# jneem/nnnoiseless

Hardware: AMD Instinct MI355X
Metric: 480-sample frames/sec (whole node) at N concurrent streams (higher is better)
Workload: dtype f32; 1 GPU; configs[2]: 65536 concurrent streams on one GPU, built-in weights.rnn, GRU as batched MFMA GEMM, synthetic 48 kHz sine+noise, 48 frame(s) per stream per step; parity=oracle pinned by the reference's golden pair (built-in model), model=built-in weights.rnn, boundary_format=f32 planar (process_frame's own), streams_per_gpu=65536, streams_total=65536, inputs_ready=True, schedule=stages, lanes=2, parallelism=streams sharded x1, one process per GPU, no data-path collective

## Files before the change

nnnoiseless_amd/csrc/nnn_kernels.hip:

```cpp
#pragma once
#include "nnn_layout.h"
#include <nnn_mfma.h>

namespace nnn {

#define NNN_TI(ptr, len, tile, lane) ((ptr) + ((size_t)(tile) * (len)) * TILE + (lane))
#define NNN_TIF(b, field, len, f, tile, lane) ((b).field + ((size_t)(b).S_pad * (size_t)(f) + (size_t)(tile) * TILE) * (size_t)(len) + (lane))

#define NNN_FRAME_SPLIT(PER)                              \
    const int frame = (int)blockIdx.x / (int)(PER);      \
    const int bx = (int)blockIdx.x - frame * (int)(PER); \
    b = frame_view(b, frame);

__device__ __forceinline__ void xcd_tile_block(int blk, int ntiles, int bpt, int &tile, int &sub)
{
    const int m8 = ntiles & ~7;
    if (blk < m8 * bpt) {
        const int xcd = blk & 7, j = blk >> 3;
        tile = xcd + 8 * (j / bpt);
        sub = j % bpt;
    } else {
        const int r = blk - m8 * bpt;
        tile = m8 + r / bpt;
        sub = r % bpt;
    }
}
__device__ __forceinline__ void xcd_tile_block_units(int blk, int ntiles, int bpt, int n, int &unit, int &tile, int &sub)
{
    const int m8 = ntiles & ~7;
    if (blk < m8 * bpt * n) {
        const int xcd = blk & 7, j = blk >> 3, tb = j / n;
        unit = j - tb * n;
        tile = xcd + 8 * (tb / bpt);
        sub = tb % bpt;
    } else {
        const int r = blk - m8 * bpt * n, per = (ntiles - m8) * bpt;
        unit = r / per;
        const int q = r - unit * per;
        tile = m8 + q / bpt;
        sub = q % bpt;
    }
}

#ifdef NNN_STAMPS
#define NNN_STAMP(b, i) do { if (blockIdx.x == 0 && blockIdx.y == 0 && threadIdx.x == 0) (b).stamps[i] = (long long)__builtin_readcyclecounter(); } while (0)
#define NNN_STAMPW(b, i, cond) do { if (blockIdx.x == 0 && (threadIdx.x & 63) == 0 && (cond)) (b).stamps[i] = (long long)__builtin_readcyclecounter(); } while (0)
#ifndef NNN_WFSTAMP_PHASE
#define NNN_WFSTAMP_PHASE 1
#endif
#else
#define NNN_STAMP(b, i) do { } while (0)
#define NNN_STAMPW(b, i, cond) do { } while (0)
#endif

#ifdef __HIPCC__
#define NNN_CONSTANT static __constant__
#else
#define NNN_CONSTANT __constant__
#endif
NNN_CONSTANT int kEband[NB] = {0, 1, 2, 3, 4, 5, 6, 7, 8, 10, 12, 14, 16, 20, 24, 28, 34, 40, 48, 60, 78, 100};
NNN_CONSTANT int kSecondCheck[16] = {0, 0, 3, 2, 3, 2, 5, 2, 3, 2, 3, 2, 5, 2, 3, 2};

template <int FMT> __device__ __forceinline__ float pcm_load(const char *p)
{
    if (FMT == PCM_I16) return (float)ld_global<short>(p);
    const float v = ld_global<float>(p);
    return FMT == PCM_F32_UNIT ? v * 32768.0f : v;
}
__device__ __forceinline__ short pcm_to_i16(float v) { return (short)roundf(fminf(fmaxf(v, -32768.0f), 32767.0f)); }
__device__ __forceinline__ float pcm_to_unit(float v)
{
    v = v / 32768.0f;
    if (v < -1.0f) v = -1.0f;
    if (v > 1.0f) v = 1.0f;
    return v;
}
__device__ __forceinline__ void pcm_store(char *p, int fmt, float v)
{
    if (fmt == PCM_I16) *(short *)p = pcm_to_i16(v);
    else *(float *)p = fmt == PCM_F32_UNIT ? pcm_to_unit(v) : v;
}
#ifndef NNN_HP_CH
#define NNN_HP_CH 32
#endif
constexpr int HP_CH = NNN_HP_CH;
// ... 571 lines not shown
    const float x0 = NNN_TI(b.xlp0, b.nslot, tile, lane)[(size_t)slot * TILE];
    float a1[1];
    if (wave == 0) lpc_chains<0, 1, LPC_CHW>(base, x0, a1);
    else if (wave == 1) lpc_chains<1, 1, LPC_CHW>(base, x0, a1);
    else if (wave == 2) lpc_chains<2, 1, LPC_CHW>(base, x0, a1);
    else if (wave == 3) lpc_chains<3, 1, LPC_CHW>(base, x0, a1);
    else lpc_chains<4, 1, LPC_CHW>(base, x0, a1);
    acs[wave][lane] = a1[0];
    __syncthreads();
    if (wave != 0) return;
    float ac[5];
#pragma unroll
    for (int k = 0; k < 5; k++) ac[k] = acs[k][lane];
    lpc_finish(b, tile, lane, slot, ac);
}

constexpr int PK_SPB = 16;
constexpr int PK_WAVES = 8;
constexpr int PK_T = 64 * PK_WAVES;
#ifndef NNN_PK_LC
#define NNN_PK_LC 13
#endif
constexpr int PK_LC = NNN_PK_LC;
constexpr int PK_NG = (NLAG1 + PK_LC - 1) / PK_LC;
static_assert((PK_LC & 1) && PK_NG <= 4 * 8, "odd group size: neighbouring groups start on different row parities");
constexpr int PK_XW = (PK_NG + 3) / 4;
constexpr int PK_JB = 8;
constexpr int PK_NP = PK_LC / 2;
constexpr int PK_NT = PK_JB / 2 + PK_NP;
static_assert((PK_NG - 1) * PK_LC + 239 + PK_JB + PK_LC < XLP / 2, "the window stays inside the even rows");
constexpr int PK_KMAX = 12;
constexpr int PK_NE = 1 + 2 * (PK_KMAX - 1);
constexpr int PK_NSLOT = PK_NE + 2;
constexpr int PK_NC = 36;

constexpr int PK_HALF = (XLP / 2) * PK_SPB;
constexpr int PK_ODD = PK_HALF + 16;
__device__ __forceinline__ int pk_at(int r, int s) { return ((r & 1) ? PK_ODD : 0) + (r >> 1) * PK_SPB + s; }


struct BestPitch {
    float best_num, second_num, best_den, second_den;
    int best, second;
    __device__ void init() { best_num = -1.0f; second_num = -1.0f; best_den = 0.0f; second_den = 0.0f; best = 0; second = 1; }
    __device__ __forceinline__ void update(int i, float corr, float y_sq_norm) {
        const float num = corr * corr;
        const bool in = corr > 0.0f && num * second_den > second_num * y_sq_norm;
        const bool top = in && num * best_den > best_num * y_sq_norm;
        const bool mid = in && !top;
        second_num = top ? best_num : (mid ? num : second_num);
        second_den = top ? best_den : (mid ? y_sq_norm : second_den);
        second = top ? best : (mid ? i : second);
        best_num = top ? num : best_num;
        best_den = top ? y_sq_norm : best_den;
        best = top ? i : best;
    }
    __device__ __forceinline__ void update_sq(int i, float num, float y_sq_norm) {
        const bool in = num * second_den > second_num * y_sq_norm;
        if (!wave_any(in)) return;
        const bool top = in && num * best_den > best_num * y_sq_norm;
        const bool mid = in && !top;
        second_num = top ? best_num : (mid ? num : second_num);
        second_den = top ? best_den : (mid ? y_sq_norm : second_den);
        second = top ? best : (mid ? i : second);
        best_num = top ? num : best_num;
        best_den = top ? y_sq_norm : best_den;
// ... 26 lines not shown
constexpr int PK_RMAX = 24;
constexpr int PK_CAP = 384;
constexpr int PK_PLW = XLP / 2 + 8;
constexpr float PK_EPS = 0.0083f;
struct PkCert {
    float denck[PK_SPB][PK_DCK];
    float bsum[PK_SPB][27];
    unsigned mask[PK_SPB][5];
    unsigned count, full, pad_[2];
    unsigned short list[PK_CAP];
    float slotv[PK_SPB][PK_RMAX], slotd[PK_SPB][PK_RMAX];
    int slotl[PK_SPB][PK_RMAX];
    alignas(16) unsigned short plane[(PK_SPB / 2) * PK_PLW + 16];
};
struct alignas(16) PkLds {
    float pb[PK_ODD + PK_HALF];
    float ckf[PK_NCKF][PK_SPB];
    float cky[PK_NCKY][PK_SPB];
    union {
        struct { float xc[NLAG1][PK_SPB], ysq[NLAG1][PK_SPB]; } c;
        PkCert a;
        struct {
            float part[PK_NC][4][PK_SPB];
            float yy[32][PK_SPB];
            float ye[10][PK_SPB];
            int cand[32][PK_SPB];
            int lo[2][PK_SPB];
            int tsel[PK_SPB];
            float xx[PK_SPB], lgain[PK_SPB];
            int t0[PK_SPB], pprev[PK_SPB];
            float kxy[16][PK_SPB], kyy[16][PK_SPB], kg[16][PK_SPB];
            int kpass[16][PK_SPB];
            int any_refine;
        } f;
    } u;
};
static_assert(sizeof(PkLds) <= 80 * 1024, "two blocks per CU");
static_assert(offsetof(PkLds, ckf) % 16 == 0 && offsetof(PkLds, u) % 16 == 0 && offsetof(PkCert, plane) % 16 == 0 && (PK_PLW * 2) % 16 == 0, "16-byte fragment reads");
static_assert(sizeof(float) * (PK_NCKF + PK_NCKY) * PK_SPB >= sizeof(unsigned short) * (PK_SPB / 2) * PK_PLW + 32, "the first eight planes fit over the check points");

constexpr int PK_CH = 32, PK_NCH = XLP / PK_CH;
static_assert(PK_NCH * PK_CH == XLP && PK_NCH * PK_SPB <= PK_T, "");

__device__ __forceinline__ void pk_window_load(const Buffers &b, const StepParams *sp, int tile, int q0, int tid, float (&v)[PK_CH],
                                               float (&fir)[5])
{
    const int col = tid & 15, ch = tid >> 4;
    if (ch >= PK_NCH) {
#pragma unroll
        for (int i = 0; i < PK_CH; i++) v[i] = 0.0f;
#pragma unroll
        for (int i = 0; i < 5; i++) fir[i] = 0.0f;
        return;
    }
    const int slot = sp->slot;
    {
        const float *lp = NNN_TI(b.lpc, b.nslot * 10, tile, q0 + col) + (size_t)(slot * 10) * TILE;
#pragma unroll
        for (int i = 0; i < 5; i++) fir[i] = lp[(size_t)(5 + i) * TILE];
    }
    const float *base = b.dec + ((size_t)tile * dec_len(b.nslot) + (size_t)dec_base(slot, b.nslot)) * TILE + q0;
    const unsigned off = (unsigned)(ch * PK_CH) * TILE + (unsigned)col;
#pragma unroll
    for (int i = 0; i < PK_CH; i++) v[i] = base[off + (unsigned)i * TILE];
    if (ch == 0) v[0] = NNN_TI(b.xlp0, b.nslot, tile, q0 + col)[(size_t)slot * TILE];
}

template <int NCAND>
// ... 230 lines not shown
}

__device__ __forceinline__ float pk_dot240(const float *xp, const float *yp)
{
    float c = 0.0f;
    v2f xa[4], ya[4], xb[4], yb[4];
#define NNN_LD(X, Y, J) do { _Pragma("unroll") for (int i_ = 0; i_ < 4; i_++) { \
        X[i_] = mk2(xp[((J) + 2 * i_) * PK_SPB], xp[((J) + 2 * i_ + 1) * PK_SPB]); Y[i_] = mk2(yp[((J) + 2 * i_) * PK_SPB], yp[((J) + 2 * i_ + 1) * PK_SPB]); } } while (0)
#define NNN_ACC(X, Y) do { _Pragma("unroll") for (int i_ = 0; i_ < 4; i_++) { const v2f pr_ = pk_mul(X[i_], Y[i_]); c = sadd(c, pr_.x); c = sadd(c, pr_.y); } } while (0)
    NNN_LD(xa, ya, 0);
#pragma nounroll
    for (int j = 0; j < 224; j += 16) {
        NNN_LD(xb, yb, j + 8);
        NNN_ACC(xa, ya);
        NNN_LD(xa, ya, j + 16);
        NNN_ACC(xb, yb);
    }
    NNN_LD(xb, yb, 232);
    NNN_ACC(xa, ya);
    NNN_ACC(xb, yb);
#undef NNN_LD
#undef NNN_ACC
    return c;
}

constexpr int PK_SEG_FS = 120;
#ifndef NNN_PK_SEG_F1
#define NNN_PK_SEG_F1 44
#endif
constexpr int PK_SEG_F1 = NNN_PK_SEG_F1;
static_assert(PK_SEG_F1 % 2 == 0 && PK_SEG_F1 <= PK_FINE_K, "");


template <bool HELD> __device__ __forceinline__ void xt_rider(const Buffers &b, const StepParams *sp, int rb, void *lds);

#ifndef NNN_PK_MINWAVES
#define NNN_PK_MINWAVES 4
#endif
template <bool LPC, bool HELD = false>
__global__ void __launch_bounds__(PK_T, NNN_PK_MINWAVES) k_pitch(Buffers b, const StepParams *sp0, int g, int chain, int seq0, unsigned tbase, int lpc_here_,
                                                                 int riders)
{
    __shared__ PkLds L;
    const int lpc_here = LPC ? lpc_here_ : 0;
    if (riders > 0 && (int)blockIdx.x >= riders) {
        xt_rider<HELD>(b, sp0, (int)blockIdx.x - riders, &L);
        return;
    }
    const int wave = __builtin_amdgcn_readfirstlane((int)(threadIdx.x >> 6)), lane0 = threadIdx.x & 63;
    int lane = lane0, s = lane & 15, q = lane >> 4;
    int item = (int)blockIdx.x;
    if (chain) {
        if (threadIdx.x == 0) L.u.f.any_refine = (int)(ticket_take(b.ticket) - tbase);
        __syncthreads();
        item = __builtin_amdgcn_readfirstlane(L.u.f.any_refine);
        __syncthreads();
    }
    const int per = b.S_pad / PK_SPB;
    const int f_begin = chain ? item / per : 0, f_end = chain ? f_begin + 1 : g;
    int tile, sub_;
    xcd_tile_block(item - f_begin * per, b.NT, TILE / PK_SPB, tile, sub_);
    const int q0 = sub_ * PK_SPB;
    if (tile * TILE + q0 >= b.S) return;
    static_assert(PK_SPB == 16, "the block's bits of the tile's word are read as one little-endian 16-bit value");
    if (HELD && b.live && ((const unsigned short *)b.live)[tile * (TILE / PK_SPB) + sub_] == 0) return;
    const int min_period = PITCH_MIN / 2, max_period = PITCH_MAX / 2;
    const bool dec_lane = wave == 0 && lane0 < PK_SPB;
    int last_period = 0;
    float last_gain = 0.0f;
    if (dec_lane && f_begin == 0) {
        last_period = NNN_TI(b.last_period, 1, tile, q0 + s)[0];
        last_gain = NNN_TI(b.last_gain, 1, tile, q0 + s)[0];
    }
    const float head_c0 = (lpc_here == 2 && wave < 5 && lane0 < PK_SPB) ? b.lpc_head[((size_t)tile * 5 + wave) * TILE + q0 + lane0] : 0.0f;
    float win[PK_CH], fir[5];
    pk_window_load(b, sp0 + f_begin, tile, q0, (int)threadIdx.x, win, fir);
    for (int f = f_begin; f < f_end; f++) {
        lane = launder_v(lane0);
        s = lane & 15;
        q = lane >> 4;
        const int sl = q0 + s;
        NNN_STAMP(b, 0);
        const int tid = 64 * wave + lane, col = tid & 15, ch = tid >> 4;
        const int qi = ((q & 1) << 1) | (q >> 1);
        const int chc = ch < PK_NCH ? ch : PK_NCH - 1;
        float *chE = L.pb + (chc * (PK_CH / 2)) * PK_SPB + col, *chO = chE + PK_ODD;
        if (ch < PK_NCH) {
#pragma unroll
            for (int m = 0; m < PK_CH / 2; m++) { chE[m * PK_SPB] = win[2 * m]; chO[m * PK_SPB] = win[2 * m + 1]; }
        }
        __syncthreads();
        NNN_STAMP(b, 1);
        if (lpc_here) {
            float *acs = &L.u.c.xc[0][0], *firs = &L.u.c.xc[8][0];
            if (wave < 5 && lane < PK_SPB) {
                const float *pbs = L.pb + lane;
                const int blk0 = lpc_here == 2 ? LPC_HEAD_BLK : 0;
                const float c0 = head_c0;
                float a;
                if (wave == 0) a = pk_autocorr<0>(pbs, blk0, c0);
// ... 35 lines not shown
                for (int m = 0; m < PK_CH / 2; m++) {
                    const v2f VE0 = mk2(v[2 * m], v[2 * m + 1]), VO0 = mk2(v[2 * m + 1], v[2 * m + 2]);
                    const v2f VE1 = mk2(v[2 * m + 2], v[2 * m + 3]), VO1 = mk2(v[2 * m + 3], v[2 * m + 4]);
                    const v2f VE2 = mk2(v[2 * m + 4], v[2 * m + 5]), VO2 = mk2(v[2 * m + 5], v[2 * m + 6]);
                    v2f o = pk_add(VO2, pk_mul_bx(N01, VE2));
                    o = pk_add(o, pk_mul_by(N01, VO1));
                    o = pk_add(o, pk_mul_bx(N23, VE1));
                    o = pk_add(o, pk_mul_by(N23, VO0));
                    o = pk_add(o, pk_mul_bx(N4, VE0));
                    if (tap) { tap[(size_t)(2 * m) * TILE] = o.x; tap[(size_t)(2 * m + 1) * TILE] = o.y; }
                    chE[m * PK_SPB] = o.x;
                    chO[m * PK_SPB] = o.y;
                }
            }
            if (ch < PK_NCH) {
                const float *ce = L.pb + launder_v((chc * (PK_CH / 2)) * PK_SPB + col);
                unsigned *pl = (unsigned *)((col < PK_SPB / 2 ? (unsigned short *)&L.ckf[0][0] : L.u.a.plane) + (col & 7) * PK_PLW + (PK_CH / 2) * ch);
                unsigned nz = 0;
                float bs = 0.0f;
#pragma unroll
                for (int m = 0; m < PK_CH / 2; m += 2) {
                    const float e0 = ce[m * PK_SPB], e1 = ce[(m + 1) * PK_SPB];
                    pl[m >> 1] = pk_bf16_rn(e0, e1);
                    bs += e0 * e0;
                    bs += e1 * e1;
                    nz |= (__float_as_uint(e0) | __float_as_uint(e1)) << 1;
                }
                L.u.a.bsum[col][ch] = (nz != 0 && bs < 0x1p-120f) ? 0x1p-120f : bs;
            }
            if (tid < PK_SPB * 5 + 2) (&L.u.a.mask[0][0])[tid] = 0u;
        }
        __syncthreads();
        NNN_STAMP(b, 4);
        const float *pE = L.pb + s, *pO = pE + PK_ODD;
        const int li = lane & 15, kg = lane >> 4;
        const int cs = lane >> 2, cq = lane & 3;
        const float *pcs = L.pb + cs;
        const int wv = launder_s(wave);
        float chain_y = 0.0f;
        auto search = [&](auto ns_, const int s0) {
            constexpr int NS = decltype(ns_)::value;
            f32x4 cacc[NS];
            unsigned m0[4], m7[4];
#pragma unroll
            for (int w = 0; w < 4; w++) {
                const int n0 = li - 8 * kg, n1 = 16 + li - 8 * kg;
                m0[w] = (2 * w >= n0 ? 0xffffu : 0u) | (2 * w + 1 >= n0 ? 0xffff0000u : 0u);
                m7[w] = (2 * w < n1 ? 0xffffu : 0u) | (2 * w + 1 < n1 ? 0xffff0000u : 0u);
            }
            const unsigned sh = (unsigned)(li & 1) * 16u;
            const char *pl[NS], *pa[NS];
#pragma unroll
            for (int u = 0; u < NS; u++) {
                const int sq = s0 + 5 * u;
                pl[u] = (const char *)((sq < PK_SPB / 2 ? (const unsigned short *)&L.ckf[0][0] : L.u.a.plane) + (sq & 7) * PK_PLW);
                pa[u] = pl[u] + ((384 + 16 * kg - 2 * li) & ~3);
                pl[u] += 16 * kg + 32 * li;
                cacc[u] = f32x4{0.0f, 0.0f, 0.0f, 0.0f};
            }
#pragma unroll
            for (int t = 0; t < 8; t++) {
#pragma unroll
                for (int u = 0; u < NS; u++) {
                    const uint4 bq = *(const uint4 *)(pl[u] + 64 * t);
                    const unsigned *d = (const unsigned *)(pa[u] + 64 * t);
                    const unsigned d0 = d[0], d1 = d[1], d2 = d[2], d3 = d[3], d4 = d[4];
// ... 94 lines not shown
                if (tot != 0) {
                    unsigned base = 0;
                    if (lane == 0) base = lds_add_u32(&L.u.a.count, tot);
                    base = __float_as_uint(lane_value(__uint_as_float(base), 0));
                    want_full |= base + tot > (unsigned)PK_CAP;
#pragma unroll
                    for (int r = 0; r < 4; r++) {
                        const int Lr = 4 * kg + r + 16 * li;
                        const unsigned ix = base + lane_rank(bal[r], lane);
                        if (keep[r] && ix < (unsigned)PK_CAP) {
                            L.u.a.list[ix] = (unsigned short)((sq << 8) | Lr);
                            lds_or_u32(&L.u.a.mask[sq][Lr >> 5], 1u << (Lr & 31));
                        }
                        base += (unsigned)__builtin_popcountll(bal[r]);
                    }
                }
                want_full |= ((cfl >> (4 + u)) & 1u) != 0 || tot > (unsigned)PK_RMAX;
            }
            if (lane == 0 && (want_full || b.taps == 1)) L.u.a.full = 1u;
        };
        if (wv < 5) search(std::integral_constant<int, 3>(), wv);
        else if (wv == 7) {
            chain_y = pk_chain_coarse_start(pcs, cq);
            chain_y = pk_chain_coarse(pcs, cq, chain_y, 0, PK_COARSE_K, L.u.a.denck[cs]);
            NNN_STAMPW(b, 3, true);
        } else if (wv == 5) {
            chain_y = pk_chain_fine_start(pcs, cq, 1.0f, 0, PK_SEG_FS);
            NNN_STAMPW(b, 28, true);
        } else if (wv == 6) {
            chain_y = pk_chain_yy_start(pcs, cq);
            NNN_STAMPW(b, 29, true);
            search(std::integral_constant<int, 1>(), 15);
        }
        __syncthreads();
        NNN_STAMP(b, 5);
        const bool full = L.u.a.full != 0;
        const unsigned nsurv = L.u.a.count;
        if (full) {
            __syncthreads();
            const int grp = 4 * wave + q;
            if (grp < PK_NG) {
                const int L0 = PK_LC * grp;
                const float *yb = L.pb + L0 * PK_SPB + s, *xb = L.pb + 192 * PK_SPB + s;
                v2f acc2[PK_NP], PE[PK_NT], PO[PK_NT];
                float acc1 = 0.0f;
#pragma unroll
                for (int n = 0; n < PK_NP; n++) acc2[n] = mk2(0.0f, 0.0f);
#pragma unroll
                for (int t = 0; t < PK_NT - PK_JB / 2; t++) {
                    PE[t] = mk2(yb[(2 * t) * PK_SPB], yb[(2 * t + 1) * PK_SPB]);
                    PO[t] = mk2(yb[(2 * t + 1) * PK_SPB], yb[(2 * t + 2) * PK_SPB]);
                }
#pragma unroll 5
                for (int j = 0; j < 240; j += PK_JB) {
                    const float *yj = yb + j * PK_SPB, *xj = xb + j * PK_SPB;
                    v2f X[PK_JB / 2];
#pragma unroll
                    for (int t = 0; t < PK_JB / 2; t++) X[t] = mk2(xj[(2 * t) * PK_SPB], xj[(2 * t + 1) * PK_SPB]);
#pragma unroll
                    for (int t = PK_NT - PK_JB / 2; t < PK_NT; t++) {
                        PE[t] = mk2(yj[(2 * t) * PK_SPB], yj[(2 * t + 1) * PK_SPB]);
                        PO[t] = mk2(yj[(2 * t + 1) * PK_SPB], yj[(2 * t + 2) * PK_SPB]);
                    }
#pragma unroll
                    for (int k = 0; k < PK_JB; k++) {
                        const v2f xp2 = X[k >> 1];
#pragma unroll
// ... 31 lines not shown
#pragma unroll
                    for (int i = 0; i < 8; i++) ysq += v[i] * v[i];
                }
#pragma nounroll
                for (int i0 = 0; i0 < NLAG1; i0 += 7) {
                    float a[7], d[7];
#pragma unroll
                    for (int i = 0; i < 7; i++) { a[i] = pE[(i0 + i + 240) * PK_SPB]; d[i] = pE[(i0 + i) * PK_SPB]; }
#pragma unroll
                    for (int i = 0; i < 7; i++) {
                        L.u.c.ysq[i0 + i][s] = ysq;
                        ysq += a[i] * a[i] - d[i] * d[i];
                        ysq = fmaxf(ysq, 1.0f);
                    }
                }
            }
            __syncthreads();
        }
        NNN_STAMP(b, 63);
        int lo1 = 0, lo2 = 0;
        if (wv == 5) chain_y = pk_chain_fine(pcs, cq, cs, chain_y, 0, PK_SEG_F1, L.ckf);
        else if (wv == 6) {
            if (cq == 0) L.cky[0][cs] = chain_y;
            chain_y = pk_chain_yy(pcs, cq, cs, chain_y, 0, PK_YY_B, L.cky);
        } else if (wv != 7 && !full) {
#pragma nounroll
            for (unsigned e0 = 64u * (unsigned)wv; e0 < nsurv; e0 += 64u * 5u) {
                const unsigned en = e0 + (unsigned)lane;
                if (en < nsurv) {
                    const unsigned ent = L.u.a.list[en];
                    const int se = (int)(ent >> 8), Le = (int)(ent & 255u);
                    const float *xp = L.pb + 192 * PK_SPB + se, *yp = L.pb + Le * PK_SPB + se;
                    const float c = pk_dot240(xp, yp);
                    const unsigned *mk = L.u.a.mask[se];
                    int rk = 0;
#pragma unroll
                    for (int w = 0; w < 5; w++) {
                        const unsigned mw = mk[w], below = w < (Le >> 5) ? mw : (w == (Le >> 5) ? mw & ((1u << (Le & 31)) - 1u) : 0u);
                        rk += __builtin_popcount(below);
                    }
                    float dy = L.u.a.denck[se][Le >> 2];
                    {
                        const float *yq = L.pb + (Le & ~3) * PK_SPB + se;
                        float ra[3], rd[3];
#pragma unroll
                        for (int i = 0; i < 3; i++) { ra[i] = yq[(i + 240) * PK_SPB]; rd[i] = yq[i * PK_SPB]; }
#pragma unroll
                        for (int i = 0; i < 3; i++) {
                            const float yn = fmaxf(dy + (ra[i] * ra[i] - rd[i] * rd[i]), 1.0f);
                            dy = i < (Le & 3) ? yn : dy;
                        }
                    }
                    L.u.a.slotv[se][rk] = c;
                    L.u.a.slotl[se][rk] = Le;
                    L.u.a.slotd[se][rk] = dy;
                    if (b.taps) NNN_TIF(b, xc1, NLAG1, f, tile, q0 + se)[(size_t)Le * TILE] = c;
                }
            }
        }
        if (full) {
            if (wv == 5) chain_y = pk_chain_fine(pcs, cq, cs, chain_y, PK_SEG_F1, PK_FINE_K, L.ckf);
            if (dec_lane) {
                BestPitch bp;
                bp.init();
                float c[7], e[7];
#pragma unroll
                for (int i = 0; i < 7; i++) { c[i] = L.u.c.xc[i][s]; e[i] = L.u.c.ysq[i][s]; }
#pragma nounroll
                for (int i0 = 0; i0 < NLAG1; i0 += 7) {
                    float cn[7], en[7];
                    const int i1 = i0 + 7 < NLAG1 ? i0 + 7 : i0;
#pragma unroll
                    for (int i = 0; i < 7; i++) { cn[i] = L.u.c.xc[i1 + i][s]; en[i] = L.u.c.ysq[i1 + i][s]; }
#pragma unroll
                    for (int i = 0; i < 7; i++) bp.update_sq(i0 + i, c[i], e[i]);
#pragma unroll
                    for (int i = 0; i < 7; i++) { c[i] = cn[i]; e[i] = en[i]; }
                }
                if (b.taps) {
                    int *o = (int *)NNN_TIF(b, best1, 2, f, tile, sl);
                    o[0] = bp.best;
                    o[TILE] = bp.second;
                }
                lo1 = 2 * bp.best - 2;
                lo2 = 2 * bp.second - 2;
                NNN_STAMP(b, 61);
            }
        } else {
            __syncthreads();
            NNN_STAMP(b, 27);
            if (wv == 5) chain_y = pk_chain_fine(pcs, cq, cs, chain_y, PK_SEG_F1, PK_FINE_K, L.ckf);
            if (wave == 0) {
                BestPitch bp;
                bp.init();
                int ns = 0;
#pragma unroll
                for (int w = 0; w < 5; w++) ns += lane < PK_SPB ? __builtin_popcount(L.u.a.mask[s][w]) : 0;
                float nc = 0.0f, nd = 1.0f;
                int nl = 0;
                if (ns > 0) { nl = L.u.a.slotl[s][0]; nc = L.u.a.slotv[s][0]; nd = L.u.a.slotd[s][0]; }
                for (int k = 0; wave_ballot(k < ns) != 0ull; k++) {
                    const int cl = nl;
                    const float cc = nc, cd = nd;
                    if (k + 1 < ns) { nl = L.u.a.slotl[s][k + 1]; nc = L.u.a.slotv[s][k + 1]; nd = L.u.a.slotd[s][k + 1]; }
                    if (k < ns) bp.update(cl, cc, cd);
                }
                if (dec_lane) {
                    if (b.taps) {
                        int *o = (int *)NNN_TIF(b, best1, 2, f, tile, sl);
                        o[0] = bp.best;
                        o[TILE] = bp.second;
                    }
                    lo1 = 2 * bp.best - 2;
                    lo2 = 2 * bp.second - 2;
                }
                NNN_STAMP(b, 61);
            }
        }
        if (wave == 0) wave_lds_sync();
        if (dec_lane) {
            L.u.f.lo[0][s] = lo1;
            L.u.f.lo[1][s] = lo2;
            if (s == 0) L.u.f.any_refine = 0;
        }
        __syncthreads();
        NNN_STAMP(b, 6);
        if (wave < 5) {
            const int la = L.u.f.lo[0][s] + wave, lb = L.u.f.lo[1][s] + wave;
            const bool va = la >= 0 && la < NLAG2, vb = lb >= 0 && lb < NLAG2;
            const int yr[2] = {va ? la : 0, vb ? lb : 0};
            float acc[2];
            pk_inner<2>(L.pb, s, qi, yr, acc);
            L.u.f.part[wave][qi][s] = acc[0];
            L.u.f.part[5 + wave][qi][s] = acc[1];
        } else if (wave == 5) {
            if (q < 2) {
                const int lo = L.u.f.lo[q][s], first = lo > 0 ? lo : 0;
                const int i0 = (first < NLAG2 ? first : NLAG2 - 1) & ~(PK_CKF - 1);
                float y = L.ckf[i0 / PK_CKF][s], ev[5] = {0.0f, 0.0f, 0.0f, 0.0f, 0.0f};
                float ra[PK_CKF + 4], rd[PK_CKF + 4];
#pragma unroll
                for (int st = 0; st < PK_CKF + 4; st++) {
                    const int i = i0 + st < NLAG2 ? i0 + st : NLAG2 - 1;
                    ra[st] = L.pb[pk_at(i + 480, s)];
                    rd[st] = L.pb[pk_at(i, s)];
                }
#pragma unroll
                for (int st = 0; st < PK_CKF + 4; st++) {
#pragma unroll
                    for (int c = 0; c < 5; c++) ev[c] = (i0 + st == lo + c) ? y : ev[c];
                    y += ra[st] * ra[st] - rd[st] * rd[st];
                    y = fmaxf(y, 1.0f);
                }
#pragma unroll
                for (int c = 0; c < 5; c++) L.u.f.ye[5 * q + c][s] = ev[c];
            }
        }
        __syncthreads();
// ... 33 lines not shown
                const float cv = (u < 5) == a_first ? xc.v[u < 5 ? u : u - 5] : xc.v[5 + (u < 5 ? u : u - 5)];
                if (on) bp.update(i, cv, e);
            }
            int offset = 0;
            if (bp.best > 0 && bp.best < NLAG2 - 1) {
                float a = xc.at(bp.best - 1), bb = xc.at(bp.best), c = xc.at(bp.best + 1);
                if (c - a > 0.7f * (bb - a)) offset = 1;
                else if (a - c > 0.7f * (bb - c)) offset = -1;
            }
            const int psr = 2 * bp.best - offset;
            if (b.taps) NNN_TIF(b, psearch, 1, f, tile, sl)[0] = psr;
            NNN_STAMP(b, 60);
            t0 = (PITCH_MAX - psr) / 2;
            if (t0 > max_period - 1) t0 = max_period - 1;
        #pragma unroll
            for (int e = 0; e < PK_NSLOT; e++) {
                int t;
                if (e == 0) t = t0;
                else if (e >= PK_NE) t = e == PK_NE ? t0 - 1 : t0 + 1;
                else {
                    const int k = 2 + (e - 1) / 2;
                    const int t1 = (2 * t0 + k) / (2 * k);
                    if ((e - 1) & 1) {
                        const int sc = kSecondCheck[k];
                        t = (k == 2) ? ((t1 + t0 > max_period) ? t0 : t0 + t1) : (2 * sc * t0 + k) / (2 * k);
                    } else t = t1;
                }
                L.u.f.cand[e][s] = t;
            }

            L.u.f.xx[s] = xx;
            L.u.f.t0[s] = t0;
        }
        __syncthreads();
        NNN_STAMP(b, 53);
        {
            const int e = 4 * wave + q;
            if (e < PK_NE) {
                const int T = L.u.f.cand[e][s], m = T / PK_CKY;
                float y = L.cky[m][s];
                float ra[PK_CKY - 1], rc[PK_CKY - 1];
#pragma unroll
                for (int st = 1; st < PK_CKY; st++) {
                    const int j = PK_CKY * m + st, jc = j <= 384 ? j : 384;
                    ra[st - 1] = L.pb[pk_at(384 - jc, s)];
                    rc[st - 1] = L.pb[pk_at(864 - jc, s)];
                }
#pragma unroll
                for (int st = 1; st < PK_CKY; st++) {
                    const float yn = y + (ra[st - 1] * ra[st - 1] - rc[st - 1] * rc[st - 1]);
                    y = PK_CKY * m + st <= T ? yn : y;
                }
                L.u.f.yy[e][s] = fmaxf(y, 0.0f);
            }
        }
        static_assert(PK_NSLOT == 25, "three slots per wave and one more");
        if (wave == 0) {
            int yr[4];
#pragma unroll
            for (int c = 0; c < 4; c++) yr[c] = max_period - L.u.f.cand[8 * c][s];
            float acc[4];
            pk_inner<4>(L.pb, s, qi, yr, acc);
#pragma unroll
            for (int c = 0; c < 4; c++) L.u.f.part[8 * c][qi][s] = acc[c];
        } else {
            int yr[3];
#pragma unroll
            for (int c = 0; c < 3; c++) yr[c] = max_period - L.u.f.cand[wave + 8 * c][s];
            float acc[3];
            pk_inner<3>(L.pb, s, qi, yr, acc);
#pragma unroll
            for (int c = 0; c < 3; c++) L.u.f.part[wave + 8 * c][qi][s] = acc[c];
        }
        pk_window_load(b, sp0 + f + 1, tile, q0, f + 1 < f_end ? tid : PK_T, win, fir);
        if (dec_lane) {
            if (chain && f > 0) {
                const int *flag = (const int *)NNN_TIF(b, pflag, 1, f - 1, tile, q0);
                const long long t_wait = realtime_ticks();
                unsigned spins = 0;
                bool lost = false;
                while (flag_read(flag) != seq0 + f - 1 && !lost) {
                    chain_pause();
                    if ((++spins & 255u) == 0 && realtime_ticks() - t_wait > b.handoff_ticks) lost = true;
                }
                if (lost) *b.fault = 1;
                last_period = NNN_TIF(b, pitch, 1, f - 1, tile, sl)[0];
                last_gain = NNN_TIF(b, pgain, 1, f - 1, tile, sl)[0];
            }
            L.u.f.pprev[s] = last_period / 2;
            L.u.f.lgain[s] = last_gain;
        }
        __syncthreads();
        NNN_STAMP(b, 54);
        if (wave < 3) {
            const int k = 2 + 4 * wave + q;
            if (k <= PK_KMAX) {
                auto ipv = [&](int e) { return L.u.f.part[e][0][s] + L.u.f.part[e][1][s] + L.u.f.part[e][2][s] + L.u.f.part[e][3][s]; };
                const int e1 = 1 + 2 * (k - 2), e2 = e1 + 1;
                const int t1 = L.u.f.cand[e1][s], t0s = L.u.f.t0[s];
                const float xxs = L.u.f.xx[s], lg = L.u.f.lgain[s];
                const float g0 = pitch_gain(ipv(0), xxs, L.u.f.yy[0][s]);
                const float xy = (ipv(e1) + ipv(e2)) / 2.0f;
                const float yy = (L.u.f.yy[e1][s] + L.u.f.yy[e2][s]) / 2.0f;
                const float g1 = pitch_gain(xy, xxs, yy);
                int d = t1 - L.u.f.pprev[s];
                if (d < 0) d = -d;
                float cont;
                if (d <= 1) cont = lg;
                else if (d <= 2 && 5 * k * k < t0s) cont = lg / 2.0f;
                else cont = 0.0f;
                float thresh;
                if (t1 < 3 * min_period) thresh = fmaxf(0.85f * g0 - cont, 0.4f);
                else if (t1 < 2 * min_period) thresh = fmaxf(0.9f * g0 - cont, 0.5f);
                else thresh = fmaxf(0.7f * g0 - cont, 0.3f);
                L.u.f.kpass[k][s] = (t1 >= min_period && g1 > thresh) ? 1 : 0;
                L.u.f.kxy[k][s] = xy;
                L.u.f.kyy[k][s] = yy;
                L.u.f.kg[k][s] = g1;
            }
        }
        __syncthreads();
        NNN_STAMP(b, 58);
        int t = 0;
        float pg = 0.0f, gg = 0.0f;
        if (dec_lane) {
            auto ipv = [&](int e) { return L.u.f.part[e][0][s] + L.u.f.part[e][1][s] + L.u.f.part[e][2][s] + L.u.f.part[e][3][s]; };
            t = t0;
            float best_xy = ipv(0), best_yy = L.u.f.yy[0][s];
            gg = pitch_gain(best_xy, xx, best_yy);
            int kw = 0;
#pragma unroll
            for (int k = 2; k <= PK_KMAX; k++) kw = L.u.f.kpass[k][s] ? k : kw;
            if (kw) {
                best_xy = L.u.f.kxy[kw][s];
                best_yy = L.u.f.kyy[kw][s];
                gg = L.u.f.kg[kw][s];
                t = L.u.f.cand[1 + 2 * (kw - 2)][s];
            }
            best_xy = fmaxf(best_xy, 0.0f);
            pg = (best_yy <= best_xy) ? 1.0f : best_xy / (best_yy + 1.0f);
            L.u.f.tsel[s] = t;
            if (t != t0) L.u.f.any_refine = 1;
        }
        __syncthreads();
        NNN_STAMP(b, 55);
        const bool refine = L.u.f.any_refine != 0;
        if (refine) {
            if (wave < 3) {
                const int yr[1] = {max_period - (L.u.f.tsel[s] + wave - 1)};
                float acc[1];
                pk_inner<1>(L.pb, s, qi, yr, acc);
                L.u.f.part[32 + wave][qi][s] = acc[0];
            }
            __syncthreads();
        }
        NNN_STAMP(b, 56);
        if (dec_lane) {
            auto ipv = [&](int e) { return L.u.f.part[e][0][s] + L.u.f.part[e][1][s] + L.u.f.part[e][2][s] + L.u.f.part[e][3][s]; };
            float x3[3];
            if (t == t0) { x3[0] = ipv(PK_NE); x3[1] = ipv(0); x3[2] = ipv(PK_NE + 1); }
            else { x3[0] = ipv(32); x3[1] = ipv(33); x3[2] = ipv(34); }
            int offset = 0;
            if (x3[2] - x3[0] > 0.7f * (x3[1] - x3[0])) offset = 1;
            else if (x3[0] - x3[2] > 0.7f * (x3[1] - x3[2])) offset = -1;
            pg = fminf(pg, gg);
            int res = 2 * t + offset;
            if (res < PITCH_MIN) res = PITCH_MIN;
            NNN_TIF(b, pitch, 1, f, tile, sl)[0] = res;
            NNN_TIF(b, pgain, 1, f, tile, sl)[0] = pg;
            last_period = res;
            last_gain = pg;
            if (chain) {
                __threadfence();
                if (lane0 == 0 && seq0 + f != b.dbg_withhold) flag_publish((int *)NNN_TIF(b, pflag, 1, f, tile, q0), seq0 + f);
            }
        }
        NNN_STAMP(b, 57);
    }
    if (dec_lane && f_end == g) {
        NNN_TI(b.last_period, 1, tile, q0 + s)[0] = last_period;
        NNN_TI(b.last_gain, 1, tile, q0 + s)[0] = last_gain;
// ... 1812 lines not shown
```

nnnoiseless_amd/csrc/nnn_batch.hip:

```cpp
#include <hip/hip_runtime.h>
#include <math.h>
#include <stdarg.h>
#include <stdio.h>
#include <stdlib.h>
#include <string.h>

#include <atomic>
#include <chrono>
#include <mutex>
#include <string>
#include <vector>

#include "../../include/nnn_batch.h"
#include "../../include/nnn_train.h"
#include "nnn_back.hip"
#include "nnn_model.h"

using namespace nnn;

static thread_local std::string g_err;
static std::recursive_mutex g_rt_mu;
constexpr int MARK_DEVICES = 64;
static std::atomic<uint64_t> g_call_mark[MARK_DEVICES];
static std::atomic<uint64_t> g_next_batch_id{1};
// ... 400 lines not shown
        }
        G.wf = !paths.rnn_rows && G.plan.dense.nb <= 2 && G.plan.vad.nb <= 2 && G.plan.noise.nb <= 3 && G.plan.dn.nb <= 6 && G.plan.vad.rec.ksteps <= WF_KS_REC &&
               G.plan.noise.rec.ksteps <= WF_KS_REC && G.plan.dn.rec.ksteps <= WF_KS_REC && G.wf_lds <= kLdsMax;
        tile0 += G.ntiles;
        h->md.nd = md.nd > h->md.nd ? md.nd : h->md.nd;
        h->md.nv = md.nv > h->md.nv ? md.nv : h->md.nv;
        h->md.nn = md.nn > h->md.nn ? md.nn : h->md.nn;
        h->md.ndn = md.ndn > h->md.ndn ? md.ndn : h->md.ndn;
    }
    const ModelDims &md = h->md;
    h->plan.rnn = new uint8_t[n_groups]();

    Buffers &b = h->b[0];
    memset(&b, 0, sizeof(b));
    b.S = h->S; b.S_pad = h->S_pad; b.NT = h->NT;
    b.nslot = h->nslot;
    b.gru_v_w = md.nv; b.gru_n_w = md.nn; b.gru_dn_w = md.ndn;
    HIPCHK(dalloc(h, &b.hist, Sp * hist_stride(h->nslot), true));
    HIPCHK(dalloc(h, &b.hp_mem, Sp * 2, true));
    HIPCHK(dalloc(h, &b.hp_last, Sp, true));
    HIPCHK(dalloc(h, &b.dec, Sp * dec_len(h->nslot), true));
    HIPCHK(dalloc(h, &b.xlp0, Sp * h->nslot, true));
    HIPCHK(dalloc(h, &b.lpc_head, (size_t)h->NT * 5 * TILE, false));
    HIPCHK(dalloc(h, &b.lpc, Sp * h->nslot * 10, false));
    HIPCHK(dalloc(h, &b.ceps_mem, Sp * CEPS_MEM * NB, true));
    HIPCHK(dalloc(h, &b.mem_id, Sp, true));
    HIPCHK(dalloc(h, &b.synth_mem, Sp * FRAME, true));
    HIPCHK(dalloc(h, &b.lastg, Sp * NB, true));
    HIPCHK(dalloc(h, &b.last_period, Sp, true));
    HIPCHK(dalloc(h, &b.last_gain, Sp, true));
    HIPCHK(dalloc(h, &b.gru_v, Sp * md.nv, true));
    HIPCHK(dalloc(h, &b.gru_n, Sp * md.nn, true));
    HIPCHK(dalloc(h, &b.gru_dn, Sp * md.ndn, true));
    HIPCHK(dalloc(h, &b.stamps, 64, false));
    {
        void *hp = nullptr, *dp = nullptr;
        HIPCHK(hipHostMalloc(&hp, sizeof(int), hipHostMallocMapped));
        *(volatile int *)hp = 0;
        HIPCHK(hipHostGetDevicePointer(&dp, hp, 0));
        h->fault_host = (volatile int *)hp;
        b.fault = (int *)dp;
    }
    HIPCHK(dalloc(h, &b.ticket, 1, false));
    b.handoff_ticks = HANDOFF_TICKS;
    HIPCHK(hipMalloc((void **)&h->sp_tab, 2 * 64 * sizeof(StepParams)));
    h->sp_tab_cap = 64;
    std::vector<float> window, dct, tansig, bin_frac;
    std::vector<float2> tw;
    std::vector<int> bin_band;
    make_tables(window, dct, tw, tansig, bin_frac, bin_band, b.wnorm);
    HIPCHK(upload(h, &b.window, window));
    {
        std::vector<float> wa(WINDOW), ws(WINDOW);
        for (int i = 0; i < WINDOW; i++) { wa[i] = window[i] * 0.5f; ws[i] = window[i] * 0.5f; }
        HIPCHK(upload(h, &b.window_a, wa));
        HIPCHK(upload(h, &b.window_s, ws));
    }
    HIPCHK(upload(h, &b.dct, dct));
    HIPCHK(upload(h, &b.tw960, tw));
    HIPCHK(upload(h, &b.tansig, tansig));
    HIPCHK(upload(h, &b.bin_frac, bin_frac));
    HIPCHK(upload(h, &b.bin_band, bin_band));
    {
        static const int E[NB] = {0, 1, 2, 3, 4, 5, 6, 7, 8, 10, 12, 14, 16, 20, 24, 28, 34, 40, 48, 60, 78, 100};
        std::vector<int> seg(192, 0);
        int ns = 0;
        for (int i = 0; i < NB - 1; i++) {
// ... 1412 lines not shown
    uint32_t *dst = (uint32_t *)host_dst;
    const size_t Sp = (size_t)h->S_pad;
    if (d.layout == 0) {
        std::vector<uint32_t> tmp(Sp * d.sub_len);
        HIPCHK(hipMemcpy(tmp.data(), p, tmp.size() * 4, hipMemcpyDeviceToHost));
        for (int s = 0; s < h->S; s++)
            for (int i = 0; i < d.len; i++)
                dst[(size_t)s * d.len + i] = tmp[((size_t)(s / TILE) * d.sub_len + d.sub_ofs + i) * TILE + s % TILE];
    } else if (d.layout == 2 || d.layout == 4) {
        std::vector<uint32_t> tmp(Sp * 2 * FSTR);
        HIPCHK(hipMemcpy(tmp.data(), p, tmp.size() * 4, hipMemcpyDeviceToHost));
        for (int s = 0; s < h->S; s++)
            for (int k = 0; k < FREQ; k++) {
                const size_t at = (size_t)s * 2 * FSTR + 2 * (size_t)(d.layout == 4 ? spectrum_index_p(k) : spectrum_index(k));
                dst[(size_t)s * d.len + 2 * k] = tmp[at];
                dst[(size_t)s * d.len + 2 * k + 1] = tmp[at + 1];
            }
    } else {
        const size_t hstr = (size_t)hist_stride(h->nslot);
        std::vector<uint32_t> tmp(Sp * hstr);
        HIPCHK(hipMemcpy(tmp.data(), p, tmp.size() * 4, hipMemcpyDeviceToHost));
        int slot = last_slot(h);
        for (int s = 0; s < h->S; s++) memcpy(dst + (size_t)s * FRAME, tmp.data() + (size_t)s * hstr + slot * FRAME, FRAME * 4);
    }
    return 0;
}

extern "C" int nnn_batch_read_stamps(nnn_batch *h, long long *dst64)
{
    NNN_RT_LOCK;
    if (!h) return fail("null batch");
    HIPCHK(hipSetDevice(h->device));
    HIPCHK(hipDeviceSynchronize());
    HIPCHK(hipMemcpy(dst64, h->b[0].stamps, 64 * sizeof(long long), hipMemcpyDeviceToHost));
    return 0;
}

extern "C" int nnn_debug_activations(int device, int act, const float *x, float *y, int n)
{
    NNN_RT_LOCK;
    if (!x || !y || n < 0 || act < 0 || act > 2) return fail("bad argument");
    HIPCHK(hipSetDevice(device));
    std::vector<float> window, dct, tansig, bin_frac;
    std::vector<float2> tw;
    std::vector<int> bin_band;
    float wnorm;
    make_tables(window, dct, tw, tansig, bin_frac, bin_band, wnorm);
    float *d = nullptr;
    HIPCHK(hipMalloc((void **)&d, (size_t)(2 * n + 256) * sizeof(float)));
    float *dx = d + 256, *dy = dx + n;
    hipError_t e = hipMemcpy(d, tansig.data(), 201 * sizeof(float), hipMemcpyHostToDevice);
    if (e == hipSuccess) e = hipMemcpy(dx, x, (size_t)n * sizeof(float), hipMemcpyHostToDevice);
    if (e == hipSuccess && n) {
        hipLaunchKernelGGL(k_activation_kat, dim3((n + 255) / 256), dim3(256), 0, (hipStream_t) nullptr, (const float *)d, (const float *)dx, dy, act, n);
        e = hipDeviceSynchronize();
    }
    if (e == hipSuccess) e = hipMemcpy(y, dy, (size_t)n * sizeof(float), hipMemcpyDeviceToHost);
    hipFree(d);
    if (e != hipSuccess) return fail("activation sweep failed: %s", hipGetErrorString(e));
    return 0;
}

extern "C" int nnn_batch_set_profiling(nnn_batch *h, int on)
{
    if (!h) return fail("null batch");
    h->profiling = on != 0;
    return 0;
// ... 307 lines not shown
```

Baseline: 76.30 million frames/s.

## Skip dead pitch-doubling candidates and compact live ones into wave work units

Before the correlation pass, the pitch kernel now works out for each stream which subharmonic candidates k can pass the min_period test. The live (k, stream) pairs are compacted into a ballot-built unit list that all waves share, so correlations are computed only for live candidates instead of every slot for every stream. Energy sums, threshold checks and the refine correlations are skipped for dead candidates and for streams whose pitch did not change. This adds LDS bookkeeping, a wave-0 ballot prologue and a dynamic loop whose trip count varies, which can unbalance the waves.

```diff
diff --git a/nnnoiseless_amd/csrc/nnn_kernels.hip b/nnnoiseless_amd/csrc/nnn_kernels.hip
--- a/nnnoiseless_amd/csrc/nnn_kernels.hip
+++ b/nnnoiseless_amd/csrc/nnn_kernels.hip
@@ -688,6 +688,7 @@
 constexpr int PK_KMAX = 12;
 constexpr int PK_NE = 1 + 2 * (PK_KMAX - 1);
 constexpr int PK_NSLOT = PK_NE + 2;
+constexpr int PK_UNITS = (PK_KMAX - 1) * PK_SPB;
 constexpr int PK_NC = 36;
 
 constexpr int PK_HALF = (XLP / 2) * PK_SPB;
@@ -780,6 +781,9 @@
             float kxy[16][PK_SPB], kyy[16][PK_SPB], kg[16][PK_SPB];
             int kpass[16][PK_SPB];
             int any_refine;
+            int klive[PK_SPB];
+            int nunit;
+            unsigned char unit[PK_UNITS];
         } f;
     } u;
 };
@@ -1662,11 +1666,27 @@
             L.u.f.xx[s] = xx;
             L.u.f.t0[s] = t0;
         }
+        if (wave == 0) {
+            int klive = 1;
+            if (dec_lane) {
+#pragma unroll
+                for (int k = 2; k <= PK_KMAX; k++) klive = ((2 * t0 + k) / (2 * k) >= min_period || b.taps) ? k : klive;
+                L.u.f.klive[s] = klive;
+            }
+            unsigned nu = 0;
+#pragma unroll
+            for (int k = 2; k <= PK_KMAX; k++) {
+                const unsigned long long bal = wave_ballot(klive >= k);
+                if (klive >= k) L.u.f.unit[nu + lane_rank(bal, lane)] = (unsigned char)((k << 4) | s);
+                nu += (unsigned)__builtin_popcountll(bal);
+            }
+            if (lane == 0) L.u.f.nunit = (int)nu;
+        }
         __syncthreads();
         NNN_STAMP(b, 53);
         {
             const int e = 4 * wave + q;
-            if (e < PK_NE) {
+            if (e < PK_NE && (e + 3) / 2 <= L.u.f.klive[s]) {
                 const int T = L.u.f.cand[e][s], m = T / PK_CKY;
                 float y = L.cky[m][s];
                 float ra[PK_CKY - 1], rc[PK_CKY - 1];
@@ -1684,23 +1704,30 @@
                 L.u.f.yy[e][s] = fmaxf(y, 0.0f);
             }
         }
-        static_assert(PK_NSLOT == 25, "three slots per wave and one more");
+        static_assert(PK_NSLOT == 25 && PK_NE == 23, "slots 0, 23, 24: t0 and its neighbours");
         if (wave == 0) {
-            int yr[4];
-#pragma unroll
-            for (int c = 0; c < 4; c++) yr[c] = max_period - L.u.f.cand[8 * c][s];
-            float acc[4];
-            pk_inner<4>(L.pb, s, qi, yr, acc);
-#pragma unroll
-            for (int c = 0; c < 4; c++) L.u.f.part[8 * c][qi][s] = acc[c];
-        } else {
-            int yr[3];
-#pragma unroll
-            for (int c = 0; c < 3; c++) yr[c] = max_period - L.u.f.cand[wave + 8 * c][s];
+            const int yr[3] = {max_period - L.u.f.cand[0][s], max_period - L.u.f.cand[PK_NE][s], max_period - L.u.f.cand[PK_NE + 1][s]};
             float acc[3];
             pk_inner<3>(L.pb, s, qi, yr, acc);
-#pragma unroll
-            for (int c = 0; c < 3; c++) L.u.f.part[wave + 8 * c][qi][s] = acc[c];
+            L.u.f.part[0][qi][s] = acc[0];
+            L.u.f.part[PK_NE][qi][s] = acc[1];
+            L.u.f.part[PK_NE + 1][qi][s] = acc[2];
+        }
+        {
+            const int nunit = __builtin_amdgcn_readfirstlane(L.u.f.nunit);
+#pragma nounroll
+            for (int u0 = PK_SPB * ((wave + PK_WAVES - 1) & (PK_WAVES - 1)); u0 < nunit; u0 += PK_SPB * PK_WAVES) {
+                const bool on = u0 + s < nunit;
+                const int ent = L.u.f.unit[on ? u0 + s : nunit - 1];
+                const int se = ent & 15, e1 = 2 * (ent >> 4) - 3;
+                const int yr[2] = {max_period - L.u.f.cand[e1][se], max_period - L.u.f.cand[e1 + 1][se]};
+                float acc[2];
+                pk_inner<2>(L.pb, se, qi, yr, acc);
+                if (on) {
+                    L.u.f.part[e1][qi][se] = acc[0];
+                    L.u.f.part[e1 + 1][qi][se] = acc[1];
+                }
+            }
         }
         pk_window_load(b, sp0 + f + 1, tile, q0, f + 1 < f_end ? tid : PK_T, win, fir);
         if (dec_lane) {
@@ -1724,7 +1751,8 @@
         NNN_STAMP(b, 54);
         if (wave < 3) {
             const int k = 2 + 4 * wave + q;
-            if (k <= PK_KMAX) {
+            if (k <= PK_KMAX && k > L.u.f.klive[s]) L.u.f.kpass[k][s] = 0;
+            else if (k <= PK_KMAX) {
                 auto ipv = [&](int e) { return L.u.f.part[e][0][s] + L.u.f.part[e][1][s] + L.u.f.part[e][2][s] + L.u.f.part[e][3][s]; };
                 const int e1 = 1 + 2 * (k - 2), e2 = e1 + 1;
                 const int t1 = L.u.f.cand[e1][s], t0s = L.u.f.t0[s];
@@ -1776,7 +1804,7 @@
         NNN_STAMP(b, 55);
         const bool refine = L.u.f.any_refine != 0;
         if (refine) {
-            if (wave < 3) {
+            if (wave < 3 && L.u.f.tsel[s] != L.u.f.t0[s]) {
                 const int yr[1] = {max_period - (L.u.f.tsel[s] + wave - 1)};
                 float acc[1];
                 pk_inner<1>(L.pb, s, qi, yr, acc);
```

Measured after the change: 74.53 million frames/s. 2.3% lower.

## Replace pitch-search block barriers with per-wave LDS handshake flags

Applied to the files above, without the earlier changes.

Replaces two __syncthreads in the pitch kernel with per-role LDS completion flags that waves poll, so each wave waits only on the producers it needs instead of the whole block. The survivor denominator computation is split out of the correlation loop and run after waiting only on the coarse-chain wave, which lets correlation work proceed without that dependency. It also adds optional role-timing stamps and doubles the stamps buffer for them. The spin-wait polling costs issue slots, and workgroup-scope relaxed atomics with wave-level syncs must order LDS correctly.

```diff
diff --git a/nnnoiseless_amd/csrc/nnn_batch.hip b/nnnoiseless_amd/csrc/nnn_batch.hip
--- a/nnnoiseless_amd/csrc/nnn_batch.hip
+++ b/nnnoiseless_amd/csrc/nnn_batch.hip
@@ -456,7 +456,7 @@
     HIPCHK(dalloc(h, &b.gru_v, Sp * md.nv, true));
     HIPCHK(dalloc(h, &b.gru_n, Sp * md.nn, true));
     HIPCHK(dalloc(h, &b.gru_dn, Sp * md.ndn, true));
-    HIPCHK(dalloc(h, &b.stamps, 64, false));
+    HIPCHK(dalloc(h, &b.stamps, 128, false));
     {
         void *hp = nullptr, *dp = nullptr;
         HIPCHK(hipHostMalloc(&hp, sizeof(int), hipHostMallocMapped));
@@ -1935,7 +1935,11 @@
     if (!h) return fail("null batch");
     HIPCHK(hipSetDevice(h->device));
     HIPCHK(hipDeviceSynchronize());
+#ifdef NNN_PK_ROLE_STAMPS
+    HIPCHK(hipMemcpy(dst64, h->b[0].stamps + 64, 64 * sizeof(long long), hipMemcpyDeviceToHost));
+#else
     HIPCHK(hipMemcpy(dst64, h->b[0].stamps, 64 * sizeof(long long), hipMemcpyDeviceToHost));
+#endif
     return 0;
 }
 
diff --git a/nnnoiseless_amd/csrc/nnn_kernels.hip b/nnnoiseless_amd/csrc/nnn_kernels.hip
--- a/nnnoiseless_amd/csrc/nnn_kernels.hip
+++ b/nnnoiseless_amd/csrc/nnn_kernels.hip
@@ -51,6 +51,11 @@
 #else
 #define NNN_STAMP(b, i) do { } while (0)
 #define NNN_STAMPW(b, i, cond) do { } while (0)
+#endif
+#if defined(NNN_STAMPS) && defined(NNN_PK_ROLE_STAMPS)
+#define NNN_STAMPR(b, i) do { if (blockIdx.x == 0 && (threadIdx.x & 63) == 0) (b).stamps[64 + (i) + (int)(threadIdx.x >> 6)] = (long long)__builtin_readcyclecounter(); } while (0)
+#else
+#define NNN_STAMPR(b, i) do { } while (0)
 #endif
 
 #ifdef __HIPCC__
@@ -782,6 +787,7 @@
             int any_refine;
         } f;
     } u;
+    unsigned hs[16];
 };
 static_assert(sizeof(PkLds) <= 80 * 1024, "two blocks per CU");
 static_assert(offsetof(PkLds, ckf) % 16 == 0 && offsetof(PkLds, u) % 16 == 0 && offsetof(PkCert, plane) % 16 == 0 && (PK_PLW * 2) % 16 == 0, "16-byte fragment reads");
@@ -1078,6 +1084,45 @@
 static_assert(PK_SEG_F1 % 2 == 0 && PK_SEG_F1 <= PK_FINE_K, "");
 
 
+__device__ __forceinline__ int pk_surv_rank(const unsigned *mk, int Le)
+{
+    int rk = 0;
+#pragma unroll
+    for (int w = 0; w < 5; w++) {
+        const unsigned mw = mk[w], below = w < (Le >> 5) ? mw : (w == (Le >> 5) ? mw & ((1u << (Le & 31)) - 1u) : 0u);
+        rk += __builtin_popcount(below);
+    }
+    return rk;
+}
+
+#ifdef __HIPCC__
+__device__ __forceinline__ void hs_store(unsigned *p, unsigned v) { __hip_atomic_store(p, v, __ATOMIC_RELAXED, __HIP_MEMORY_SCOPE_WORKGROUP); }
+__device__ __forceinline__ unsigned hs_load(const unsigned *p) { return __hip_atomic_load(p, __ATOMIC_RELAXED, __HIP_MEMORY_SCOPE_WORKGROUP); }
+#else
+static inline void hs_store(unsigned *p, unsigned v) { *p = v; }
+static inline unsigned hs_load(const unsigned *p) { return *p; }
+#endif
+__device__ __forceinline__ void pk_role_done(unsigned *word, int lane, unsigned fv)
+{
+    wave_lds_sync();
+    if (lane == 0) hs_store(word, fv);
+}
+__device__ __forceinline__ void pk_roles_wait(const unsigned *hs, unsigned need, unsigned fv)
+{
+    for (;;) {
+        bool missing = false;
+#pragma unroll
+        for (int i = 0; i < 16; i++)
+            if ((need >> i) & 1u) missing |= (int)(hs_load(hs + i) - fv) < 0;
+        if (wave_ballot(missing) == 0ull) break;
+        chain_pause();
+    }
+    wave_lds_sync();
+}
+constexpr unsigned PK_HS_LISTED = 0x005fu;
+constexpr unsigned PK_HS_COARSE = 0x8000u;
+constexpr unsigned PK_HS_SLOTS = 0x1e00u;
+
 template <bool HELD> __device__ __forceinline__ void xt_rider(const Buffers &b, const StepParams *sp, int rb, void *lds);
 
 #ifndef NNN_PK_MINWAVES
@@ -1112,6 +1157,7 @@
     if (HELD && b.live && ((const unsigned short *)b.live)[tile * (TILE / PK_SPB) + sub_] == 0) return;
     const int min_period = PITCH_MIN / 2, max_period = PITCH_MAX / 2;
     const bool dec_lane = wave == 0 && lane0 < PK_SPB;
+    if (threadIdx.x < 16) L.hs[threadIdx.x] = 0u;
     int last_period = 0;
     float last_gain = 0.0f;
     if (dec_lane && f_begin == 0) {
@@ -1213,6 +1259,7 @@
         }
         __syncthreads();
         NNN_STAMP(b, 4);
+        NNN_STAMPR(b, 48);
         const float *pE = L.pb + s, *pO = pE + PK_ODD;
         const int li = lane & 15, kg = lane >> 4;
         const int cs = lane >> 2, cq = lane & 3;
@@ -1373,7 +1420,12 @@
             NNN_STAMPW(b, 29, true);
             search(std::integral_constant<int, 1>(), 15);
         }
-        __syncthreads();
+        const unsigned fv = (unsigned)f + 1u;
+        if (wv < 5 || wv == 6) pk_role_done(&L.hs[wv], lane, fv);
+        else if (wv == 7) pk_role_done(&L.hs[15], lane, fv);
+        NNN_STAMPR(b, 0);
+        pk_roles_wait(L.hs, PK_HS_LISTED, fv);
+        NNN_STAMPR(b, 24);
         NNN_STAMP(b, 5);
         const bool full = L.u.a.full != 0;
         const unsigned nsurv = L.u.a.count;
@@ -1471,29 +1523,31 @@
                     const int se = (int)(ent >> 8), Le = (int)(ent & 255u);
                     const float *xp = L.pb + 192 * PK_SPB + se, *yp = L.pb + Le * PK_SPB + se;
                     const float c = pk_dot240(xp, yp);
-                    const unsigned *mk = L.u.a.mask[se];
-                    int rk = 0;
-#pragma unroll
-                    for (int w = 0; w < 5; w++) {
-                        const unsigned mw = mk[w], below = w < (Le >> 5) ? mw : (w == (Le >> 5) ? mw & ((1u << (Le & 31)) - 1u) : 0u);
-                        rk += __builtin_popcount(below);
-                    }
-                    float dy = L.u.a.denck[se][Le >> 2];
-                    {
-                        const float *yq = L.pb + (Le & ~3) * PK_SPB + se;
-                        float ra[3], rd[3];
-#pragma unroll
-                        for (int i = 0; i < 3; i++) { ra[i] = yq[(i + 240) * PK_SPB]; rd[i] = yq[i * PK_SPB]; }
-#pragma unroll
-                        for (int i = 0; i < 3; i++) {
-                            const float yn = fmaxf(dy + (ra[i] * ra[i] - rd[i] * rd[i]), 1.0f);
-                            dy = i < (Le & 3) ? yn : dy;
-                        }
-                    }
+                    const int rk = pk_surv_rank(L.u.a.mask[se], Le);
                     L.u.a.slotv[se][rk] = c;
                     L.u.a.slotl[se][rk] = Le;
-                    L.u.a.slotd[se][rk] = dy;
                     if (b.taps) NNN_TIF(b, xc1, NLAG1, f, tile, q0 + se)[(size_t)Le * TILE] = c;
+                }
+            }
+            NNN_STAMPR(b, 56);
+            pk_roles_wait(L.hs, PK_HS_COARSE, fv);
+#pragma nounroll
+            for (unsigned e0 = 64u * (unsigned)wv; e0 < nsurv; e0 += 64u * 5u) {
+                const unsigned en = e0 + (unsigned)lane;
+                if (en < nsurv) {
+                    const unsigned ent = L.u.a.list[en];
+                    const int se = (int)(ent >> 8), Le = (int)(ent & 255u);
+                    float dy = L.u.a.denck[se][Le >> 2];
+                    const float *yq = L.pb + (Le & ~3) * PK_SPB + se;
+                    float ra[3], rd[3];
+#pragma unroll
+                    for (int i = 0; i < 3; i++) { ra[i] = yq[(i + 240) * PK_SPB]; rd[i] = yq[i * PK_SPB]; }
+#pragma unroll
+                    for (int i = 0; i < 3; i++) {
+                        const float yn = fmaxf(dy + (ra[i] * ra[i] - rd[i] * rd[i]), 1.0f);
+                        dy = i < (Le & 3) ? yn : dy;
+                    }
+                    L.u.a.slotd[se][pk_surv_rank(L.u.a.mask[se], Le)] = dy;
                 }
             }
         }
@@ -1526,7 +1580,10 @@
                 NNN_STAMP(b, 61);
             }
         } else {
-            __syncthreads();
+            if (wv >= 1 && wv < 5) pk_role_done(&L.hs[8 + wv], lane, fv);
+            NNN_STAMPR(b, 8);
+            if (wave == 0) pk_roles_wait(L.hs, PK_HS_SLOTS, fv);
+            NNN_STAMPR(b, 32);
             NNN_STAMP(b, 27);
             if (wv == 5) chain_y = pk_chain_fine(pcs, cq, cs, chain_y, PK_SEG_F1, PK_FINE_K, L.ckf);
             if (wave == 0) {
@@ -1562,7 +1619,9 @@
             L.u.f.lo[1][s] = lo2;
             if (s == 0) L.u.f.any_refine = 0;
         }
+        NNN_STAMPR(b, 16);
         __syncthreads();
+        NNN_STAMPR(b, 40);
         NNN_STAMP(b, 6);
         if (wave < 5) {
             const int la = L.u.f.lo[0][s] + wave, lb = L.u.f.lo[1][s] + wave;
```

New measurement: 75.83 million frames/s before, 75.66 million frames/s after, median of 2. About the same (-0.2%).
